# leotimus/binary-recommendation

Measured on AMD Instinct MI355X. Metric: (user,item) pairs/sec at batch 65536 dim 64, higher is better.
Workload: dtype f32; 1 GPU; NeuMF-A full training step (trainers/NFC_plain.py graph: 4 embeddings, 128->100->50->10->1, BCE, Keras-Adam adam_dense), embed_dim=64, 1000000 users x 100000 items per GPU, batch 65536 per GPU, uniform ids; global_batch=65536, parallelism=single GPU, steps_per_graph_launch=4, optimizer=adam_dense (deferred replay)

## Files before the change

### binary-recommendation_amd/csrc/stamps.h

```cpp
#pragma once
#include "common.h"

namespace br {

#ifdef BR_STAMPS
constexpr int kStampSlots = 12;
__device__ unsigned long long* g_stamp_buf = nullptr;
#define BR_STAMP_DECL unsigned long long stamps_[kStampSlots] = {0, 0, 0, 0, 0, 0, 0, 0, 0, 0, 0, 0}
#define BR_STAMP(i)                                                                             \
  do {                                                                                          \
    __builtin_amdgcn_sched_barrier(0);                                                          \
    unsigned long long t_;                                                                      \
    asm volatile("s_memtime %0\n\ts_waitcnt lgkmcnt(0)" : "=s"(t_)::"memory");                  \
    if (stamps_[i] == 0) stamps_[i] = t_;                                                       \
    __builtin_amdgcn_sched_barrier(0);                                                          \
  } while (0)
#define BR_STAMP_RT(i)                                                                          \
  do {                                                                                          \
    unsigned long long t_;                                                                      \
    asm volatile("s_memrealtime %0\n\ts_waitcnt lgkmcnt(0)" : "=s"(t_)::"memory");              \
    stamps_[i] = t_;                                                                            \
  } while (0)
#define BR_STAMP_FLUSH(widx)                                                                    \
  do {                                                                                          \
    if ((threadIdx.x & 63) == 0 && g_stamp_buf)                                                 \
      for (int i_ = 0; i_ < kStampSlots; ++i_) g_stamp_buf[(size_t)(widx) * kStampSlots + i_] = stamps_[i_]; \
  } while (0)
#else
#define BR_STAMP_DECL
#define BR_STAMP(i)
#define BR_STAMP_RT(i)
#define BR_STAMP_FLUSH(widx)
#endif

}
```

### binary-recommendation_amd/csrc/tail_mfma.hip

```cpp
#include "dense.h"

namespace br {

using f32x4 = __attribute__((ext_vector_type(4))) float;

constexpr int kTmThreads = 512;
constexpr int kTmWaves = kTmThreads / 64;
constexpr int kTmRep = BR_STAT_REPLICAS;
constexpr int kTmPatchLd = 20;
constexpr int kTmKT = 4;

__device__ __forceinline__ f32x4 mfma16t(float a, float b, f32x4 c) {
  return __builtin_amdgcn_mfma_f32_16x16x4f32(a, b, c, 0, 0, 0);
}
__device__ __forceinline__ float keep_bit_t(float x, uint32_t w, uint32_t pos) {
  return __int_as_float(__float_as_int(x) & __builtin_amdgcn_sbfe((int)w, pos, 1u));
}

struct TailTile {
  float4 av[kTmKT];
  uint32_t ka[2];
  float xr[4][kTmKT], dv[4], yv[4];
  uint32_t kc[4][2];
  int vm[4];
};
__device__ __forceinline__ void tail_load_tile(TailTile& t, const TailMArgs& a, int64_t tile, int c16, int g) {
  const int64_t batch = a.batch, rbase = tile << 4;
  const int n2 = a.n2;
  const int64_t arow = rbase + c16 < batch ? rbase + c16 : batch - 1;
  const float* pa = a.a2 + arow * a.lda2 + 4 * g;
#pragma unroll
  for (int j = 0; j < kTmKT; ++j) t.av[j] = *reinterpret_cast<const float4*>(16 * j + 4 * g < n2 ? pa + 16 * j : pa - 4 * g);
  t.ka[0] = t.ka[1] = 0xFFFFFFFFu;
  if (a.keep) { t.ka[0] = a.keep[arow * a.kw]; t.ka[1] = a.keep[arow * a.kw + (a.kw > 1 ? 1 : 0)]; }
#pragma unroll
  for (int r = 0; r < 4; ++r) {
    const int64_t row = rbase + 4 * g + r;
    t.vm[r] = row < batch ? -1 : 0;
    const int64_t rc = row < batch ? row : batch - 1;
    const float* px = a.a2 + rc * a.lda2;
#pragma unroll
    for (int kt = 0; kt < kTmKT; ++kt) { const int k = kt * 16 + c16; t.xr[r][kt] = px[k < n2 ? k : 0]; }
    t.kc[r][0] = a.keep ? a.keep[rc * a.kw] : 0xFFFFFFFFu;
    t.kc[r][1] = a.keep ? a.keep[rc * a.kw + (a.kw > 1 ? 1 : 0)] : 0xFFFFFFFFu;
    t.dv[r] = a.dot[rc];
    t.yv[r] = a.labels[rc];
  }
}

__global__ __launch_bounds__(kTmThreads, 2) void neumf_tail_mfma_kernel(const TailMArgs a) {
  __shared__ __attribute__((aligned(16))) float Wf[4 * 4 * 16 * 4];
  __shared__ __attribute__((aligned(16))) float Wb[64 * 16];
  __shared__ float cst[4][64];
  __shared__ __attribute__((aligned(16))) float hv[2][16];
  __shared__ __attribute__((aligned(16))) float patches[kTmWaves][16 * kTmPatchLd];
  __shared__ float wsum[kTmWaves][64 * 16];
  __shared__ float wcol[kTmWaves][2][16 + 2];
  __shared__ double wbn[2][64];
  __shared__ double wmet[kTmWaves][BR_METRIC_SUMS];
  const int lane = threadIdx.x & 63, wave = threadIdx.x >> 6;
  const int c16 = lane & 15, g = lane >> 4;
  const int n2 = a.n2, n3 = a.n3;
  const int64_t batch = a.batch;
  const int moff = a.mf_first ? 1 : 0;
  const int sigmask = a.act == BR_ACT_SIGMOID ? -1 : 0, relumask = a.act == BR_ACT_RELU ? -1 : 0;
  const float floor_ = a.act == BR_ACT_RELU ? 0.f : -__builtin_inff();

  const int64_t n_tiles = (batch + 15) >> 4;
  const int64_t tile0 = (int64_t)blockIdx.x * kTmWaves + wave;
  TailTile tt;
  if (tile0 < n_tiles) tail_load_tile(tt, a, tile0, c16, g);
  for (int t = threadIdx.x; t < 64; t += kTmThreads) {
    float sc = 0.f, sh = 0.f, mu = 0.f, rs = 0.f;
    if (t < n2) {
      if (a.stats2) {
        double s1 = 0.0, s2 = 0.0;
        for (int r = 0; r < kTmRep; ++r) { s1 += a.stats2[(size_t)r * 2 * n2 + t]; s2 += a.stats2[(size_t)r * 2 * n2 + n2 + t]; }
        const double m = s1 / a.batch_total;
        double var = s2 / a.batch_total - m * m;
        if (var < 0.0) var = 0.0;
        mu = (float)m;
        const float varf = (float)var;
        rs = 1.0f / sqrtf(varf + a.bn_eps);
        sc = a.gamma2[t] * rs;
        sh = a.beta2[t] - mu * sc;
        if (blockIdx.x == 0) {
          a.out_scale[t] = sc; a.out_shift[t] = sh; a.out_mean[t] = mu; a.out_rstd[t] = rs;
          if (a.moving_mean) {
            a.moving_mean[t] = a.moving_mean[t] * a.bn_momentum + mu * (1.0f - a.bn_momentum);
            a.moving_var[t] = a.moving_var[t] * a.bn_momentum + varf * (1.0f - a.bn_momentum);
          }
        }
      } else { sc = a.scale2[t]; sh = a.shift2[t]; mu = a.mean2[t]; rs = a.rstd2[t]; }
    }
    cst[0][t] = sc; cst[1][t] = sh; cst[2][t] = mu; cst[3][t] = rs;
    wbn[0][t] = 0.0; wbn[1][t] = 0.0;
  }
  for (int t = threadIdx.x; t < 16; t += kTmThreads) {
    hv[0][t] = t < n3 ? a.b3[t] : 0.f;
    hv[1][t] = t < n3 ? a.w4[moff + t] : 0.f;
  }
  for (int t = threadIdx.x; t < 64 * 16; t += kTmThreads) {
    const int k = t >> 4, n = t & 15;
    const float w = (k < n2 && n < n3) ? a.W3[k * n3 + n] : 0.f;
    Wb[t] = w;
    Wf[(((k >> 4) * 4 + ((k >> 2) & 3)) * 16 + n) * 4 + (k & 3)] = w;
  }
  __syncthreads();

  const float wdot = a.w4[a.mf_first ? 0 : n3], bias4 = a.b4[0];
  float* patch = patches[wave];
  f32x4 dW[kTmKT];
#pragma unroll
  for (int kt = 0; kt < kTmKT; ++kt) dW[kt] = (f32x4){0.f, 0.f, 0.f, 0.f};
  float db3 = 0.f, dw4 = 0.f, dw4dot = 0.f, db4 = 0.f;
  float isum[kTmKT], isq[kTmKT];
#pragma unroll
  for (int kt = 0; kt < kTmKT; ++kt) { isum[kt] = 0.f; isq[kt] = 0.f; }
  double s_loss = 0.0, s_se = 0.0, s_ae = 0.0, s_ok = 0.0, s_bce = 0.0, s_tp = 0.0, s_fp = 0.0, s_fn = 0.0;
  const float4 w4q = *reinterpret_cast<const float4*>(&hv[1][4 * g]);
  const float b3c = hv[0][c16], w4c = hv[1][c16];
  const float ik = a.inv_keep;

  for (int64_t tile = tile0; tile < n_tiles; tile += (int64_t)gridDim.x * kTmWaves) {
    const int64_t rbase = tile << 4;
    if (tile != tile0) tail_load_tile(tt, a, tile, c16, g);
    float4 (&av)[kTmKT] = tt.av;
    uint32_t (&ka)[2] = tt.ka;
    float (&xr)[4][kTmKT] = tt.xr;
    float (&dv)[4] = tt.dv;
    float (&yv)[4] = tt.yv;
    uint32_t (&kc)[4][2] = tt.kc;
    int (&vm)[4] = tt.vm;
    f32x4 z = (f32x4){0.f, 0.f, 0.f, 0.f};
#pragma unroll
    for (int j = 0; j < kTmKT; ++j) {
      const int k = 16 * j + 4 * g;
      const float4 sc = *reinterpret_cast<const float4*>(&cst[0][k]), sh = *reinterpret_cast<const float4*>(&cst[1][k]);
      const uint32_t w = ka[j >> 1], p0 = 16u * (j & 1) + 4u * g;
      const float t0 = keep_bit_t(fmaf(av[j].x, sc.x, sh.x), w, p0), t1 = keep_bit_t(fmaf(av[j].y, sc.y, sh.y), w, p0 + 1);
      const float t2 = keep_bit_t(fmaf(av[j].z, sc.z, sh.z), w, p0 + 2), t3 = keep_bit_t(fmaf(av[j].w, sc.w, sh.w), w, p0 + 3);
      const float4 b = *reinterpret_cast<const float4*>(Wf + ((j * 4 + g) * 16 + c16) * 4);
      z = mfma16t(t0, b.x, z); z = mfma16t(t1, b.y, z); z = mfma16t(t2, b.z, z); z = mfma16t(t3, b.w, z);
    }
    const int cm = c16 < n3 ? -1 : 0;
    float a3v[4];
#pragma unroll
    for (int r = 0; r < 4; ++r) {
      const float zz = fmaf(z[r], ik, b3c);
      const float s = __builtin_amdgcn_rcpf(1.0f + __builtin_amdgcn_exp2f(zz * -1.44269504088896340736f));
      const float m = fmaxf(zz, floor_);
      a3v[r] = __int_as_float(((__float_as_int(s) & sigmask) | (__float_as_int(m) & ~sigmask)) & cm);
      patch[(4 * g + r) * kTmPatchLd + c16] = a3v[r];
    }
    __builtin_amdgcn_wave_barrier();
    const float4 ar = *reinterpret_cast<const float4*>(patch + c16 * kTmPatchLd + 4 * g);
    __builtin_amdgcn_wave_barrier();
    f32x4 lzv = (f32x4){0.f, 0.f, 0.f, 0.f};
    lzv = mfma16t(ar.x, w4q.x, lzv); lzv = mfma16t(ar.y, w4q.y, lzv); lzv = mfma16t(ar.z, w4q.z, lzv); lzv = mfma16t(ar.w, w4q.w, lzv);
    float dzl[4];
#pragma unroll
    for (int r = 0; r < 4; ++r) {
      const float lz = lzv[r] + bias4 + dv[r] * wdot;
      const float e = expf(-fabsf(lz));
      const float rinv = 1.0f / (1.0f + e);
      const float p = lz >= 0.f ? rinv : e * rinv;
      float l, d;
      const float bce = fmaxf(lz, 0.f) - lz * yv[r] + log1pf(e);
      if (a.loss == BR_LOSS_BCE) { l = bce; d = (p - yv[r]) * a.inv_batch; }
      else { l = (p - yv[r]) * (p - yv[r]); d = 2.f * (p - yv[r]) * p * (1.f - p) * a.inv_batch; }
      dzl[r] = __int_as_float(__float_as_int(d) & vm[r]);
      if (c16 == 0 && vm[r]) {
        const int64_t row = rbase + 4 * g + r;
        a.logit[row] = lz; a.prob[row] = p; a.ddot[row] = dzl[r] * wdot;
        s_loss += (double)l; s_se += (double)((p - yv[r]) * (p - yv[r])); s_ae += (double)fabsf(p - yv[r]);
        const bool pp = p > 0.5f, yp = yv[r] > 0.5f;
        s_ok += (pp == yp) ? 1.0 : 0.0;
        s_bce += (double)bce; s_tp += (pp && yp) ? 1.0 : 0.0; s_fp += (pp && !yp) ? 1.0 : 0.0; s_fn += (!pp && yp) ? 1.0 : 0.0;
        dw4dot = fmaf(dzl[r], dv[r], dw4dot);
        db4 += dzl[r];
      }
    }
    float dz3[4];
#pragma unroll
    for (int r = 0; r < 4; ++r) {
      const float ds = a3v[r] * (1.f - a3v[r]);
      const float dr = a3v[r] > 0.f ? 1.f : 0.f;
      const float dl = __int_as_float((__float_as_int(ds) & sigmask) | (__float_as_int(dr) & relumask) | (0x3f800000 & ~(sigmask | relumask)));
      dz3[r] = __int_as_float(__float_as_int(dzl[r] * w4c * dl) & cm);
      dw4 = fmaf(dzl[r], a3v[r], dw4);
      db3 += dz3[r];
      patch[(4 * g + r) * kTmPatchLd + c16] = dz3[r];
      if (a.a3 && c16 < n3 && vm[r]) a.a3[(rbase + 4 * g + r) * n3 + c16] = a3v[r];
    }
    __builtin_amdgcn_wave_barrier();
    const float4 dzr = *reinterpret_cast<const float4*>(patch + c16 * kTmPatchLd + 4 * g);
    __builtin_amdgcn_wave_barrier();
    const bool row_ok = rbase + c16 < batch;
    float* ghrow = a.gh2 + (rbase + (row_ok ? c16 : 0)) * a.ldgh2 + 4 * g;
#pragma unroll
    for (int kt = 0; kt < kTmKT; ++kt) {
      const int k = kt * 16 + c16;
      const float4 b = *reinterpret_cast<const float4*>(Wb + k * 16 + 4 * g);
      f32x4 gh = (f32x4){0.f, 0.f, 0.f, 0.f};
      gh = mfma16t(dzr.x, b.x, gh); gh = mfma16t(dzr.y, b.y, gh); gh = mfma16t(dzr.z, b.z, gh); gh = mfma16t(dzr.w, b.w, gh);
      const float sck = cst[0][k], shk = cst[1][k], muk = cst[2][k], rsk = cst[3][k];
#pragma unroll
      for (int r = 0; r < 4; ++r) {
        const uint32_t w = kc[r][kt >> 1], pos = 16u * (kt & 1) + c16;
        const float dh = keep_bit_t(gh[r] * ik, w, pos);
        isum[kt] += dh;
        isq[kt] = fmaf(dh, (xr[r][kt] - muk) * rsk, isq[kt]);
        patch[(4 * g + r) * kTmPatchLd + c16] = dh;
        const float tx = keep_bit_t(fmaf(xr[r][kt], sck, shk), w, pos);
        dW[kt] = mfma16t(tx, dz3[r], dW[kt]);
      }
      __builtin_amdgcn_wave_barrier();
      const float4 o = *reinterpret_cast<const float4*>(patch + c16 * kTmPatchLd + 4 * g);
      __builtin_amdgcn_wave_barrier();
      if (row_ok && kt * 16 + 4 * g < n2) *reinterpret_cast<float4*>(ghrow + kt * 16) = o;
    }
  }

#pragma unroll
  for (int kt = 0; kt < kTmKT; ++kt) {
#pragma unroll
    for (int r = 0; r < 4; ++r) wsum[wave][(kt * 16 + 4 * g + r) * 16 + c16] = dW[kt][r];
    float sv = isum[kt], q = isq[kt];
    sv += __shfl_xor(sv, 16, 64); sv += __shfl_xor(sv, 32, 64);
    q += __shfl_xor(q, 16, 64); q += __shfl_xor(q, 32, 64);
    if (g == 0) { atomicAdd(&wbn[0][kt * 16 + c16], (double)sv); atomicAdd(&wbn[1][kt * 16 + c16], (double)q); }
  }
  {
    float v0 = db3, v1 = dw4;
    v0 += __shfl_xor(v0, 16, 64); v0 += __shfl_xor(v0, 32, 64);
    v1 += __shfl_xor(v1, 16, 64); v1 += __shfl_xor(v1, 32, 64);
    if (g == 0) { wcol[wave][0][c16] = v0; wcol[wave][1][c16] = v1; }
    float u0 = c16 == 0 ? dw4dot : 0.f, u1 = c16 == 0 ? db4 : 0.f;
    u0 = group_sum<64>(u0); u1 = group_sum<64>(u1);
    if (lane == 0) { wcol[wave][0][16] = u0; wcol[wave][0][17] = u1; }
    s_loss = wave_sum_d(s_loss); s_se = wave_sum_d(s_se); s_ae = wave_sum_d(s_ae); s_ok = wave_sum_d(s_ok);
    s_bce = wave_sum_d(s_bce); s_tp = wave_sum_d(s_tp); s_fp = wave_sum_d(s_fp); s_fn = wave_sum_d(s_fn);
    if (lane == 0) {
      wmet[wave][0] = s_loss; wmet[wave][1] = s_se; wmet[wave][2] = s_ae; wmet[wave][3] = s_ok;
      wmet[wave][4] = s_bce; wmet[wave][5] = s_tp; wmet[wave][6] = s_fp; wmet[wave][7] = s_fn;
    }
  }
  __syncthreads();
  const int64_t slab_el = (int64_t)n2 * n3 + 2 * n3 + 2;
  float* slab = a.slabs + (int64_t)blockIdx.x * slab_el;
  for (int64_t sl = (int64_t)blockIdx.x + gridDim.x; sl < a.n_slabs; sl += gridDim.x)
    for (int t = threadIdx.x; t < slab_el; t += kTmThreads) a.slabs[sl * slab_el + t] = 0.f;
  for (int t = threadIdx.x; t < 64 * 16; t += kTmThreads) {
    const int k = t >> 4, n = t & 15;
    if (k < n2 && n < n3) {
      float s = 0.f;
#pragma unroll
      for (int w = 0; w < kTmWaves; ++w) s += wsum[w][t];
      slab[k * n3 + n] = s * ik;
    }
  }
  if (threadIdx.x < 18) {
    const int t = threadIdx.x;
    float s0 = 0.f, s1 = 0.f;
#pragma unroll
    for (int w = 0; w < kTmWaves; ++w) { s0 += wcol[w][0][t]; s1 += t < 16 ? wcol[w][1][t] : 0.f; }
    if (t < n3) { slab[n2 * n3 + t] = s0; slab[n2 * n3 + n3 + moff + t] = s1; }
    if (t == 16) slab[n2 * n3 + n3 + (a.mf_first ? 0 : n3)] = s0;
    if (t == 17) slab[n2 * n3 + 2 * n3 + 1] = s0;
  }
  if (threadIdx.x >= 64 && threadIdx.x < 64 + BR_METRIC_SUMS && a.msums) {
    const int t = threadIdx.x - 64;
    double v = 0.0;
#pragma unroll
    for (int w = 0; w < kTmWaves; ++w) v += wmet[w][t];
    atomicAdd(a.msums + (size_t)(blockIdx.x & (BR_SUM_SLOTS - 1)) * BR_METRIC_SUMS + t, v);
  }
  if (a.bn_sums && threadIdx.x >= 128 && threadIdx.x < 128 + 64) {
    const int k = threadIdx.x - 128;
    if (k < n2) {
      double* rep = a.bn_sums + (size_t)(blockIdx.x % kTmRep) * 2 * n2;
      atomicAdd(rep + k, wbn[0][k]);
      atomicAdd(rep + n2 + k, wbn[1][k]);
    }
  }
}

int tail_mfma_grid(int64_t batch) {
  const int64_t t = ceil_div(ceil_div(batch > 0 ? batch : 1, 16), kTmWaves);
  return (int)(t < 1 ? 1 : (t > 256 ? 256 : t));
}
void launch_tail_mfma(const TailMArgs& a, int grid, hipStream_t s) { neumf_tail_mfma_kernel<<<(unsigned)grid, kTmThreads, 0, s>>>(a); }

}
```

Before: 210.9 million pairs/s.

## Restructure tail MFMA kernel: 1024 threads, LDS-parked tile, shared row loads

Doubles the block to 1024 threads (16 waves). Each tile's activation rows and keep masks are loaded once as float4, then parked in per-wave LDS for the backward pass, replacing the redundant per-lane strided loads of xr, kc, dot and labels. The loss epilogue is now spread across four lanes per row group, with the results broadcast through DPP, and the per-row metrics are accumulated in LDS as integer counts. BN partials are stored per wave instead of through shared double atomics, and the next tile is prefetched at the end of each iteration. The bigger block and added LDS buffers may lower occupancy, and optional timestamp probes are added behind a macro.

```diff
diff --git a/binary-recommendation_amd/csrc/stamps.h b/binary-recommendation_amd/csrc/stamps.h
--- a/binary-recommendation_amd/csrc/stamps.h
+++ b/binary-recommendation_amd/csrc/stamps.h
@@ -4,9 +4,9 @@
 namespace br {
 
 #ifdef BR_STAMPS
-constexpr int kStampSlots = 12;
+constexpr int kStampSlots = 16;
 __device__ unsigned long long* g_stamp_buf = nullptr;
-#define BR_STAMP_DECL unsigned long long stamps_[kStampSlots] = {0, 0, 0, 0, 0, 0, 0, 0, 0, 0, 0, 0}
+#define BR_STAMP_DECL unsigned long long stamps_[kStampSlots] = {}
 #define BR_STAMP(i)                                                                             \
   do {                                                                                          \
     __builtin_amdgcn_sched_barrier(0);                                                          \
@@ -21,6 +21,7 @@
     asm volatile("s_memrealtime %0\n\ts_waitcnt lgkmcnt(0)" : "=s"(t_)::"memory");              \
     stamps_[i] = t_;                                                                            \
   } while (0)
+#define BR_STAMP_WAIT_VM() asm volatile("s_waitcnt vmcnt(0)" ::: "memory")
 #define BR_STAMP_FLUSH(widx)                                                                    \
   do {                                                                                          \
     if ((threadIdx.x & 63) == 0 && g_stamp_buf)                                                 \
@@ -30,6 +31,7 @@
 #define BR_STAMP_DECL
 #define BR_STAMP(i)
 #define BR_STAMP_RT(i)
+#define BR_STAMP_WAIT_VM()
 #define BR_STAMP_FLUSH(widx)
 #endif
 
diff --git a/binary-recommendation_amd/csrc/tail_mfma.hip b/binary-recommendation_amd/csrc/tail_mfma.hip
--- a/binary-recommendation_amd/csrc/tail_mfma.hip
+++ b/binary-recommendation_amd/csrc/tail_mfma.hip
@@ -1,65 +1,73 @@
 #include "dense.h"
+#include "stamps.h"
 
 namespace br {
 
 using f32x4 = __attribute__((ext_vector_type(4))) float;
 
-constexpr int kTmThreads = 512;
+constexpr int kTmThreads = 1024;
 constexpr int kTmWaves = kTmThreads / 64;
 constexpr int kTmRep = BR_STAT_REPLICAS;
 constexpr int kTmPatchLd = 20;
+constexpr int kTmTileLd = 68;
 constexpr int kTmKT = 4;
+static_assert(16 * kTmTileLd >= 64 * 16, "the parked tile doubles as the wave's dW3 partial");
 
 __device__ __forceinline__ f32x4 mfma16t(float a, float b, f32x4 c) {
   return __builtin_amdgcn_mfma_f32_16x16x4f32(a, b, c, 0, 0, 0);
 }
 __device__ __forceinline__ float keep_bit_t(float x, uint32_t w, uint32_t pos) {
   return __int_as_float(__float_as_int(x) & __builtin_amdgcn_sbfe((int)w, pos, 1u));
+}
+template <int R>
+__device__ __forceinline__ float quad_bcast(float v) {
+  return __int_as_float(__builtin_amdgcn_update_dpp(0, __float_as_int(v), R * 0x55, 0xf, 0xf, false));
 }
 
 struct TailTile {
   float4 av[kTmKT];
   uint32_t ka[2];
-  float xr[4][kTmKT], dv[4], yv[4];
-  uint32_t kc[4][2];
-  int vm[4];
+  float dv, yv;
 };
 __device__ __forceinline__ void tail_load_tile(TailTile& t, const TailMArgs& a, int64_t tile, int c16, int g) {
-  const int64_t batch = a.batch, rbase = tile << 4;
+  const int64_t rbase = tile << 4;
   const int n2 = a.n2;
-  const int64_t arow = rbase + c16 < batch ? rbase + c16 : batch - 1;
-  const float* pa = a.a2 + arow * a.lda2 + 4 * g;
+  const int last = a.batch - rbase < 16 ? (int)(a.batch - rbase) - 1 : 15;
+  const int ar = c16 < last ? c16 : last;
+  const float* pa = a.a2 + rbase * a.lda2 + ((int64_t)ar * a.lda2 + 4 * g);
 #pragma unroll
   for (int j = 0; j < kTmKT; ++j) t.av[j] = *reinterpret_cast<const float4*>(16 * j + 4 * g < n2 ? pa + 16 * j : pa - 4 * g);
   t.ka[0] = t.ka[1] = 0xFFFFFFFFu;
-  if (a.keep) { t.ka[0] = a.keep[arow * a.kw]; t.ka[1] = a.keep[arow * a.kw + (a.kw > 1 ? 1 : 0)]; }
-#pragma unroll
-  for (int r = 0; r < 4; ++r) {
-    const int64_t row = rbase + 4 * g + r;
-    t.vm[r] = row < batch ? -1 : 0;
-    const int64_t rc = row < batch ? row : batch - 1;
-    const float* px = a.a2 + rc * a.lda2;
-#pragma unroll
-    for (int kt = 0; kt < kTmKT; ++kt) { const int k = kt * 16 + c16; t.xr[r][kt] = px[k < n2 ? k : 0]; }
-    t.kc[r][0] = a.keep ? a.keep[rc * a.kw] : 0xFFFFFFFFu;
-    t.kc[r][1] = a.keep ? a.keep[rc * a.kw + (a.kw > 1 ? 1 : 0)] : 0xFFFFFFFFu;
-    t.dv[r] = a.dot[rc];
-    t.yv[r] = a.labels[rc];
-  }
-}
-
-__global__ __launch_bounds__(kTmThreads, 2) void neumf_tail_mfma_kernel(const TailMArgs a) {
+  if (a.keep) {
+    const uint32_t* kb = a.keep + rbase * a.kw;
+    const int ko = ar * a.kw;
+    t.ka[0] = kb[ko];
+    if (a.kw > 1) t.ka[1] = kb[ko + 1];
+  }
+  const int hr = 4 * g + (c16 & 3);
+  const int hc = hr < last ? hr : last;
+  t.dv = (a.dot + rbase)[hc];
+  t.yv = (a.labels + rbase)[hc];
+}
+
+__global__ __launch_bounds__(kTmThreads) void neumf_tail_mfma_kernel(const TailMArgs a) {
   __shared__ __attribute__((aligned(16))) float Wf[4 * 4 * 16 * 4];
   __shared__ __attribute__((aligned(16))) float Wb[64 * 16];
   __shared__ float cst[4][64];
   __shared__ __attribute__((aligned(16))) float hv[2][16];
   __shared__ __attribute__((aligned(16))) float patches[kTmWaves][16 * kTmPatchLd];
-  __shared__ float wsum[kTmWaves][64 * 16];
+  __shared__ __attribute__((aligned(16))) float tiles[kTmWaves][16 * kTmTileLd];
   __shared__ float wcol[kTmWaves][2][16 + 2];
-  __shared__ double wbn[2][64];
+  __shared__ float wbn[kTmWaves][2][64];
   __shared__ double wmet[kTmWaves][BR_METRIC_SUMS];
-  const int lane = threadIdx.x & 63, wave = threadIdx.x >> 6;
-  const int c16 = lane & 15, g = lane >> 4;
+  __shared__ double lmet[kTmWaves][16][4];
+  __shared__ int lcnt[kTmWaves][16][4];
+  BR_STAMP_DECL;
+  BR_STAMP_RT(12);
+  BR_STAMP(0);
+  const int lane = threadIdx.x & 63, wave = __builtin_amdgcn_readfirstlane(threadIdx.x >> 6);
+  const int c16_ = lane & 15, g_ = lane >> 4;
+  int c16 = c16_, g = g_;
   const int n2 = a.n2, n3 = a.n3;
   const int64_t batch = a.batch;
   const int moff = a.mf_first ? 1 : 0;
@@ -67,49 +75,48 @@
   const float floor_ = a.act == BR_ACT_RELU ? 0.f : -__builtin_inff();
 
   const int64_t n_tiles = (batch + 15) >> 4;
-  const int64_t tile0 = (int64_t)blockIdx.x * kTmWaves + wave;
+  const int64_t tile0 = (int64_t)blockIdx.x * kTmWaves + wave, tstride = (int64_t)gridDim.x * kTmWaves;
   TailTile tt;
   if (tile0 < n_tiles) tail_load_tile(tt, a, tile0, c16, g);
-  for (int t = threadIdx.x; t < 64; t += kTmThreads) {
-    float sc = 0.f, sh = 0.f, mu = 0.f, rs = 0.f;
-    if (t < n2) {
-      if (a.stats2) {
-        double s1 = 0.0, s2 = 0.0;
-        for (int r = 0; r < kTmRep; ++r) { s1 += a.stats2[(size_t)r * 2 * n2 + t]; s2 += a.stats2[(size_t)r * 2 * n2 + n2 + t]; }
-        const double m = s1 / a.batch_total;
-        double var = s2 / a.batch_total - m * m;
-        if (var < 0.0) var = 0.0;
-        mu = (float)m;
-        const float varf = (float)var;
-        rs = 1.0f / sqrtf(varf + a.bn_eps);
-        sc = a.gamma2[t] * rs;
-        sh = a.beta2[t] - mu * sc;
-        if (blockIdx.x == 0) {
-          a.out_scale[t] = sc; a.out_shift[t] = sh; a.out_mean[t] = mu; a.out_rstd[t] = rs;
-          if (a.moving_mean) {
-            a.moving_mean[t] = a.moving_mean[t] * a.bn_momentum + mu * (1.0f - a.bn_momentum);
-            a.moving_var[t] = a.moving_var[t] * a.bn_momentum + varf * (1.0f - a.bn_momentum);
+  {
+    const int t = threadIdx.x, k = t >> 4, n = t & 15;
+    const float w = (k < n2 && n < n3) ? a.W3[k * n3 + n] : 0.f;
+    if (t < 64) {
+      float sc = 0.f, sh = 0.f, mu = 0.f, rs = 0.f;
+      if (t < n2) {
+        if (a.stats2) {
+          double s1 = 0.0, s2 = 0.0;
+          for (int r = 0; r < kTmRep; ++r) { s1 += a.stats2[(size_t)r * 2 * n2 + t]; s2 += a.stats2[(size_t)r * 2 * n2 + n2 + t]; }
+          const double m = s1 / a.batch_total;
+          double var = s2 / a.batch_total - m * m;
+          if (var < 0.0) var = 0.0;
+          mu = (float)m;
+          const float varf = (float)var;
+          rs = 1.0f / sqrtf(varf + a.bn_eps);
+          sc = a.gamma2[t] * rs;
+          sh = a.beta2[t] - mu * sc;
+          if (blockIdx.x == 0) {
+            a.out_scale[t] = sc; a.out_shift[t] = sh; a.out_mean[t] = mu; a.out_rstd[t] = rs;
+            if (a.moving_mean) {
+              a.moving_mean[t] = a.moving_mean[t] * a.bn_momentum + mu * (1.0f - a.bn_momentum);
+              a.moving_var[t] = a.moving_var[t] * a.bn_momentum + varf * (1.0f - a.bn_momentum);
+            }
           }
-        }
-      } else { sc = a.scale2[t]; sh = a.shift2[t]; mu = a.mean2[t]; rs = a.rstd2[t]; }
-    }
-    cst[0][t] = sc; cst[1][t] = sh; cst[2][t] = mu; cst[3][t] = rs;
-    wbn[0][t] = 0.0; wbn[1][t] = 0.0;
-  }
-  for (int t = threadIdx.x; t < 16; t += kTmThreads) {
-    hv[0][t] = t < n3 ? a.b3[t] : 0.f;
-    hv[1][t] = t < n3 ? a.w4[moff + t] : 0.f;
-  }
-  for (int t = threadIdx.x; t < 64 * 16; t += kTmThreads) {
-    const int k = t >> 4, n = t & 15;
-    const float w = (k < n2 && n < n3) ? a.W3[k * n3 + n] : 0.f;
+        } else { sc = a.scale2[t]; sh = a.shift2[t]; mu = a.mean2[t]; rs = a.rstd2[t]; }
+      }
+      cst[0][t] = sc; cst[1][t] = sh; cst[2][t] = mu; cst[3][t] = rs;
+    }
+    if (t < 16) {
+      hv[0][t] = t < n3 ? a.b3[t] : 0.f;
+      hv[1][t] = t < n3 ? a.w4[moff + t] : 0.f;
+    }
     Wb[t] = w;
     Wf[(((k >> 4) * 4 + ((k >> 2) & 3)) * 16 + n) * 4 + (k & 3)] = w;
   }
   __syncthreads();
+  BR_STAMP(1);
 
   const float wdot = a.w4[a.mf_first ? 0 : n3], bias4 = a.b4[0];
-  float* patch = patches[wave];
   f32x4 dW[kTmKT];
 #pragma unroll
   for (int kt = 0; kt < kTmKT; ++kt) dW[kt] = (f32x4){0.f, 0.f, 0.f, 0.f};
@@ -117,32 +124,43 @@
   float isum[kTmKT], isq[kTmKT];
 #pragma unroll
   for (int kt = 0; kt < kTmKT; ++kt) { isum[kt] = 0.f; isq[kt] = 0.f; }
-  double s_loss = 0.0, s_se = 0.0, s_ae = 0.0, s_ok = 0.0, s_bce = 0.0, s_tp = 0.0, s_fp = 0.0, s_fn = 0.0;
+  if (c16 < 4) {
+    double* lm = lmet[wave][4 * g + c16];
+    int* lc = lcnt[wave][4 * g + c16];
+    lm[0] = 0.0; lm[1] = 0.0; lm[2] = 0.0; lm[3] = 0.0; lc[0] = 0; lc[1] = 0; lc[2] = 0; lc[3] = 0;
+  }
   const float4 w4q = *reinterpret_cast<const float4*>(&hv[1][4 * g]);
   const float b3c = hv[0][c16], w4c = hv[1][c16];
   const float ik = a.inv_keep;
 
-  for (int64_t tile = tile0; tile < n_tiles; tile += (int64_t)gridDim.x * kTmWaves) {
+  for (int64_t tile = tile0; tile < n_tiles; tile += tstride) {
+    asm volatile("" ::: "memory");
+    c16 = c16_; g = g_;
+    asm volatile("" : "+v"(c16), "+v"(g));
+    const int hq = c16 & 3;
+    float* patch = patches[wave];
+    float* tl = tiles[wave];
     const int64_t rbase = tile << 4;
-    if (tile != tile0) tail_load_tile(tt, a, tile, c16, g);
-    float4 (&av)[kTmKT] = tt.av;
-    uint32_t (&ka)[2] = tt.ka;
-    float (&xr)[4][kTmKT] = tt.xr;
-    float (&dv)[4] = tt.dv;
-    float (&yv)[4] = tt.yv;
-    uint32_t (&kc)[4][2] = tt.kc;
-    int (&vm)[4] = tt.vm;
+    const int rows = batch - rbase < 16 ? (int)(batch - rbase) : 16;
+    BR_STAMP_WAIT_VM();
+    if (tile == tile0) BR_STAMP(2); else BR_STAMP(6);
     f32x4 z = (f32x4){0.f, 0.f, 0.f, 0.f};
 #pragma unroll
     for (int j = 0; j < kTmKT; ++j) {
       const int k = 16 * j + 4 * g;
       const float4 sc = *reinterpret_cast<const float4*>(&cst[0][k]), sh = *reinterpret_cast<const float4*>(&cst[1][k]);
-      const uint32_t w = ka[j >> 1], p0 = 16u * (j & 1) + 4u * g;
-      const float t0 = keep_bit_t(fmaf(av[j].x, sc.x, sh.x), w, p0), t1 = keep_bit_t(fmaf(av[j].y, sc.y, sh.y), w, p0 + 1);
-      const float t2 = keep_bit_t(fmaf(av[j].z, sc.z, sh.z), w, p0 + 2), t3 = keep_bit_t(fmaf(av[j].w, sc.w, sh.w), w, p0 + 3);
+      const float4 av = tt.av[j];
+      const uint32_t w = tt.ka[j >> 1], p0 = 16u * (j & 1) + 4u * g;
+      const float t0 = keep_bit_t(fmaf(av.x, sc.x, sh.x), w, p0), t1 = keep_bit_t(fmaf(av.y, sc.y, sh.y), w, p0 + 1);
+      const float t2 = keep_bit_t(fmaf(av.z, sc.z, sh.z), w, p0 + 2), t3 = keep_bit_t(fmaf(av.w, sc.w, sh.w), w, p0 + 3);
       const float4 b = *reinterpret_cast<const float4*>(Wf + ((j * 4 + g) * 16 + c16) * 4);
       z = mfma16t(t0, b.x, z); z = mfma16t(t1, b.y, z); z = mfma16t(t2, b.z, z); z = mfma16t(t3, b.w, z);
-    }
+      *reinterpret_cast<float4*>(tl + c16 * kTmTileLd + 16 * j + 4 * g) = av;
+    }
+    if (g == 0) { tl[c16 * kTmTileLd + 64] = __uint_as_float(tt.ka[0]); tl[c16 * kTmTileLd + 65] = __uint_as_float(tt.ka[1]); }
+    const float dv = tt.dv, yv = tt.yv;
+    if (tile == tile0) BR_STAMP(3); else BR_STAMP(7);
+    __builtin_amdgcn_sched_barrier(0);
     const int cm = c16 < n3 ? -1 : 0;
     float a3v[4];
 #pragma unroll
@@ -158,29 +176,34 @@
     __builtin_amdgcn_wave_barrier();
     f32x4 lzv = (f32x4){0.f, 0.f, 0.f, 0.f};
     lzv = mfma16t(ar.x, w4q.x, lzv); lzv = mfma16t(ar.y, w4q.y, lzv); lzv = mfma16t(ar.z, w4q.z, lzv); lzv = mfma16t(ar.w, w4q.w, lzv);
-    float dzl[4];
-#pragma unroll
-    for (int r = 0; r < 4; ++r) {
-      const float lz = lzv[r] + bias4 + dv[r] * wdot;
+    float dzh;
+    {
+      const int hr = 4 * g + hq;
+      const int vmh = hr < rows ? -1 : 0;
+      const float lzs = hq == 0 ? lzv[0] : hq == 1 ? lzv[1] : hq == 2 ? lzv[2] : lzv[3];
+      const float lz = lzs + bias4 + dv * wdot;
       const float e = expf(-fabsf(lz));
       const float rinv = 1.0f / (1.0f + e);
       const float p = lz >= 0.f ? rinv : e * rinv;
       float l, d;
-      const float bce = fmaxf(lz, 0.f) - lz * yv[r] + log1pf(e);
-      if (a.loss == BR_LOSS_BCE) { l = bce; d = (p - yv[r]) * a.inv_batch; }
-      else { l = (p - yv[r]) * (p - yv[r]); d = 2.f * (p - yv[r]) * p * (1.f - p) * a.inv_batch; }
-      dzl[r] = __int_as_float(__float_as_int(d) & vm[r]);
-      if (c16 == 0 && vm[r]) {
-        const int64_t row = rbase + 4 * g + r;
-        a.logit[row] = lz; a.prob[row] = p; a.ddot[row] = dzl[r] * wdot;
-        s_loss += (double)l; s_se += (double)((p - yv[r]) * (p - yv[r])); s_ae += (double)fabsf(p - yv[r]);
-        const bool pp = p > 0.5f, yp = yv[r] > 0.5f;
-        s_ok += (pp == yp) ? 1.0 : 0.0;
-        s_bce += (double)bce; s_tp += (pp && yp) ? 1.0 : 0.0; s_fp += (pp && !yp) ? 1.0 : 0.0; s_fn += (!pp && yp) ? 1.0 : 0.0;
-        dw4dot = fmaf(dzl[r], dv[r], dw4dot);
-        db4 += dzl[r];
+      const float bce = fmaxf(lz, 0.f) - lz * yv + log1pf(e);
+      if (a.loss == BR_LOSS_BCE) { l = bce; d = (p - yv) * a.inv_batch; }
+      else { l = (p - yv) * (p - yv); d = 2.f * (p - yv) * p * (1.f - p) * a.inv_batch; }
+      dzh = __int_as_float(__float_as_int(d) & vmh);
+      if (c16 < 4 && vmh) {
+        (a.logit + rbase)[hr] = lz; (a.prob + rbase)[hr] = p; (a.ddot + rbase)[hr] = dzh * wdot;
+        double* lm = lmet[wave][hr];
+        int* lc = lcnt[wave][hr];
+        lm[0] += (double)l; lm[1] += (double)((p - yv) * (p - yv)); lm[2] += (double)fabsf(p - yv); lm[3] += (double)bce;
+        const bool pp = p > 0.5f, yp = yv > 0.5f;
+        lc[0] += (pp == yp) ? 1 : 0; lc[1] += (pp && yp) ? 1 : 0; lc[2] += (pp && !yp) ? 1 : 0; lc[3] += (!pp && yp) ? 1 : 0;
+        dw4dot = fmaf(dzh, dv, dw4dot);
+        db4 += dzh;
       }
     }
+    const float dzl[4] = {quad_bcast<0>(dzh), quad_bcast<1>(dzh), quad_bcast<2>(dzh), quad_bcast<3>(dzh)};
+    if (tile == tile0) BR_STAMP(4); else BR_STAMP(8);
+    __builtin_amdgcn_sched_barrier(0);
     float dz3[4];
 #pragma unroll
     for (int r = 0; r < 4; ++r) {
@@ -191,13 +214,14 @@
       dw4 = fmaf(dzl[r], a3v[r], dw4);
       db3 += dz3[r];
       patch[(4 * g + r) * kTmPatchLd + c16] = dz3[r];
-      if (a.a3 && c16 < n3 && vm[r]) a.a3[(rbase + 4 * g + r) * n3 + c16] = a3v[r];
+      if (a.a3 && c16 < n3 && 4 * g + r < rows) (a.a3 + rbase * n3)[(4 * g + r) * n3 + c16] = a3v[r];
     }
     __builtin_amdgcn_wave_barrier();
     const float4 dzr = *reinterpret_cast<const float4*>(patch + c16 * kTmPatchLd + 4 * g);
     __builtin_amdgcn_wave_barrier();
-    const bool row_ok = rbase + c16 < batch;
-    float* ghrow = a.gh2 + (rbase + (row_ok ? c16 : 0)) * a.ldgh2 + 4 * g;
+    const bool row_ok = c16 < rows;
+    float* ghrow = a.gh2 + rbase * a.ldgh2 + ((int64_t)(row_ok ? c16 : 0) * a.ldgh2 + 4 * g);
+    const float* tr = tl + 4 * g * kTmTileLd;
 #pragma unroll
     for (int kt = 0; kt < kTmKT; ++kt) {
       const int k = kt * 16 + c16;
@@ -207,56 +231,69 @@
       const float sck = cst[0][k], shk = cst[1][k], muk = cst[2][k], rsk = cst[3][k];
 #pragma unroll
       for (int r = 0; r < 4; ++r) {
-        const uint32_t w = kc[r][kt >> 1], pos = 16u * (kt & 1) + c16;
+        const uint32_t w = __float_as_uint(tr[r * kTmTileLd + 64 + (kt >> 1)]), pos = 16u * (kt & 1) + c16;
+        const float x = tr[r * kTmTileLd + k];
         const float dh = keep_bit_t(gh[r] * ik, w, pos);
         isum[kt] += dh;
-        isq[kt] = fmaf(dh, (xr[r][kt] - muk) * rsk, isq[kt]);
+        isq[kt] = fmaf(dh, (x - muk) * rsk, isq[kt]);
         patch[(4 * g + r) * kTmPatchLd + c16] = dh;
-        const float tx = keep_bit_t(fmaf(xr[r][kt], sck, shk), w, pos);
+        const float tx = keep_bit_t(fmaf(x, sck, shk), w, pos);
         dW[kt] = mfma16t(tx, dz3[r], dW[kt]);
       }
       __builtin_amdgcn_wave_barrier();
       const float4 o = *reinterpret_cast<const float4*>(patch + c16 * kTmPatchLd + 4 * g);
       __builtin_amdgcn_wave_barrier();
       if (row_ok && kt * 16 + 4 * g < n2) *reinterpret_cast<float4*>(ghrow + kt * 16) = o;
-    }
-  }
-
+      __builtin_amdgcn_sched_barrier(0);
+    }
+    if (tile == tile0) BR_STAMP(5); else BR_STAMP(9);
+    if (tile + tstride < n_tiles) tail_load_tile(tt, a, tile + tstride, c16, g);
+  }
+
+  const int ce = threadIdx.x & 15, ge = (threadIdx.x >> 4) & 3;
 #pragma unroll
   for (int kt = 0; kt < kTmKT; ++kt) {
 #pragma unroll
-    for (int r = 0; r < 4; ++r) wsum[wave][(kt * 16 + 4 * g + r) * 16 + c16] = dW[kt][r];
+    for (int r = 0; r < 4; ++r) tiles[wave][(kt * 16 + 4 * ge + r) * 16 + ce] = dW[kt][r];
     float sv = isum[kt], q = isq[kt];
     sv += __shfl_xor(sv, 16, 64); sv += __shfl_xor(sv, 32, 64);
     q += __shfl_xor(q, 16, 64); q += __shfl_xor(q, 32, 64);
-    if (g == 0) { atomicAdd(&wbn[0][kt * 16 + c16], (double)sv); atomicAdd(&wbn[1][kt * 16 + c16], (double)q); }
+    if (ge == 0) { wbn[wave][0][kt * 16 + ce] = sv; wbn[wave][1][kt * 16 + ce] = q; }
   }
   {
     float v0 = db3, v1 = dw4;
     v0 += __shfl_xor(v0, 16, 64); v0 += __shfl_xor(v0, 32, 64);
     v1 += __shfl_xor(v1, 16, 64); v1 += __shfl_xor(v1, 32, 64);
-    if (g == 0) { wcol[wave][0][c16] = v0; wcol[wave][1][c16] = v1; }
-    float u0 = c16 == 0 ? dw4dot : 0.f, u1 = c16 == 0 ? db4 : 0.f;
+    if (ge == 0) { wcol[wave][0][ce] = v0; wcol[wave][1][ce] = v1; }
+    float u0 = ce < 4 ? dw4dot : 0.f, u1 = ce < 4 ? db4 : 0.f;
     u0 = group_sum<64>(u0); u1 = group_sum<64>(u1);
     if (lane == 0) { wcol[wave][0][16] = u0; wcol[wave][0][17] = u1; }
-    s_loss = wave_sum_d(s_loss); s_se = wave_sum_d(s_se); s_ae = wave_sum_d(s_ae); s_ok = wave_sum_d(s_ok);
-    s_bce = wave_sum_d(s_bce); s_tp = wave_sum_d(s_tp); s_fp = wave_sum_d(s_fp); s_fn = wave_sum_d(s_fn);
+    const bool hl = ce < 4;
+    const double* lm = lmet[wave][4 * ge + (ce & 3)];
+    const int* lc = lcnt[wave][4 * ge + (ce & 3)];
+    double s_loss = hl ? lm[0] : 0.0, s_se = hl ? lm[1] : 0.0, s_ae = hl ? lm[2] : 0.0, s_bce = hl ? lm[3] : 0.0;
+    int c0 = hl ? lc[0] : 0, c1 = hl ? lc[1] : 0, c2 = hl ? lc[2] : 0, c3 = hl ? lc[3] : 0;
+    for (int off : {1, 2, 16, 32}) {
+      s_loss += __shfl_xor(s_loss, off, 64); s_se += __shfl_xor(s_se, off, 64); s_ae += __shfl_xor(s_ae, off, 64); s_bce += __shfl_xor(s_bce, off, 64);
+      c0 += __shfl_xor(c0, off, 64); c1 += __shfl_xor(c1, off, 64); c2 += __shfl_xor(c2, off, 64); c3 += __shfl_xor(c3, off, 64);
+    }
     if (lane == 0) {
-      wmet[wave][0] = s_loss; wmet[wave][1] = s_se; wmet[wave][2] = s_ae; wmet[wave][3] = s_ok;
-      wmet[wave][4] = s_bce; wmet[wave][5] = s_tp; wmet[wave][6] = s_fp; wmet[wave][7] = s_fn;
+      wmet[wave][0] = s_loss; wmet[wave][1] = s_se; wmet[wave][2] = s_ae; wmet[wave][3] = (double)c0;
+      wmet[wave][4] = s_bce; wmet[wave][5] = (double)c1; wmet[wave][6] = (double)c2; wmet[wave][7] = (double)c3;
     }
   }
   __syncthreads();
+  BR_STAMP(10);
   const int64_t slab_el = (int64_t)n2 * n3 + 2 * n3 + 2;
   float* slab = a.slabs + (int64_t)blockIdx.x * slab_el;
   for (int64_t sl = (int64_t)blockIdx.x + gridDim.x; sl < a.n_slabs; sl += gridDim.x)
     for (int t = threadIdx.x; t < slab_el; t += kTmThreads) a.slabs[sl * slab_el + t] = 0.f;
-  for (int t = threadIdx.x; t < 64 * 16; t += kTmThreads) {
-    const int k = t >> 4, n = t & 15;
+  {
+    const int t = threadIdx.x, k = t >> 4, n = t & 15;
     if (k < n2 && n < n3) {
       float s = 0.f;
 #pragma unroll
-      for (int w = 0; w < kTmWaves; ++w) s += wsum[w][t];
+      for (int w = 0; w < kTmWaves; ++w) s += tiles[w][t];
       slab[k * n3 + n] = s * ik;
     }
   }
@@ -279,11 +316,17 @@
   if (a.bn_sums && threadIdx.x >= 128 && threadIdx.x < 128 + 64) {
     const int k = threadIdx.x - 128;
     if (k < n2) {
+      double s0 = 0.0, s1 = 0.0;
+#pragma unroll
+      for (int w = 0; w < kTmWaves; ++w) { s0 += (double)wbn[w][0][k]; s1 += (double)wbn[w][1][k]; }
       double* rep = a.bn_sums + (size_t)(blockIdx.x % kTmRep) * 2 * n2;
-      atomicAdd(rep + k, wbn[0][k]);
-      atomicAdd(rep + n2 + k, wbn[1][k]);
-    }
-  }
+      atomicAdd(rep + k, s0);
+      atomicAdd(rep + n2 + k, s1);
+    }
+  }
+  BR_STAMP(11);
+  BR_STAMP_RT(13);
+  BR_STAMP_FLUSH(blockIdx.x * kTmWaves + wave);
 }
 
 int tail_mfma_grid(int64_t batch) {
```

Result: no change. 212.8 million pairs/s (median of 6 runs) (+0.9%).
